# sephiroce/srf

Hardware: AMD Instinct MI355X
Metric: acoustic frames/sec through SRF (123-d fbank, 3-iter DR) at 1/2/4/8 MI355X (higher is better)
Workload: dtype fp32; 1 GPU; wsj_c4: SRF L=6 PH=CH=16 DIM=32 LPAD=RPAD=2 DR iter=3, train step (fwd+bwd+allreduce+Adam); utterances_per_gpu=28, frames_per_utterance=800, global_batch=28, parallelism=dp1, launch=hipgraph (fwd+CTC+bwd)

## Files before the change

### include/srf.h

```cpp
#ifndef SRF_H_
#define SRF_H_
#include <stddef.h>

#ifdef __cplusplus
extern "C" {
#endif

int srf_version(void);
const char* srf_last_error(void);

int srf_route_dr_auto_chunks(int B, int T, int N, int din, int lpad, int rpad, int J, int dout);
int srf_route_dr_split_table(int B, int T, int N, int din, int lpad, int rpad, int J, int dout, int n_chunks,
                             int* info, int* table, int capacity);
int srf_route_dr_set_bal_placement(int on);
int srf_route_dr_split_placement(int B, int T, int N, int din, int lpad, int rpad, int J, int dout, int n_chunks,
                                 int* block_to_wg, int capacity);
size_t srf_route_dr_saved_floats(int B, int T, int J, int dout, int iters);
size_t srf_route_dr_fwd_workspace(int B, int T, int N, int din, int lpad, int rpad, int J, int dout, int iters,
                                  int n_chunks);
size_t srf_route_dr_bwd_workspace(int B, int T, int N, int din, int lpad, int rpad, int J, int dout, int iters,
                                  int n_chunks);
int srf_route_dr_fwd(const float* emb, const float* W, const float* bias, int B, int T, int N, int din, int lpad,
                     int rpad, int J, int dout, int iters, int mask_first, int n_chunks, float* v_out,
                     float* saved, void* workspace, size_t workspace_bytes, void* stream);
size_t srf_route_dr_coupling_floats(int B, int T, int N, int din, int lpad, int rpad, int J, int dout, int iters);
#define SRF_DR_LAYOUT_N 17
int srf_route_dr_operand_layout(int B, int T, int N, int din, int lpad, int rpad, int J, int dout, int iters,
                                long long* out);
int srf_route_dr_fwd_ex(const float* emb, const float* W, const float* bias, int B, int T, int N, int din, int lpad,
                        int rpad, int J, int dout, int iters, int mask_first, int n_chunks, float* v_out,
                        float* saved, float* couplings, void* workspace, size_t workspace_bytes, void* stream);
int srf_route_dr_bwd_ex(const float* emb, const float* W, const float* bias, int B, int T, int N, int din, int lpad,
                        int rpad, int J, int dout, int iters, int mask_first, int n_chunks, const float* saved,
                        const float* couplings, const float* g_v, float* g_emb, float* g_W, float* g_bias,
                        void* workspace, size_t workspace_bytes, void* stream);
int srf_route_dr_bwd_weights_ex(const float* emb, int B, int T, int N, int din, int lpad, int rpad, int J, int dout,
                                int iters, int mask_first, int n_chunks, const float* saved, const float* couplings,
                                float* g_W, float* g_bias, void* workspace, size_t workspace_bytes, void* stream);
int srf_route_dr_bwd_data_ex(const float* emb, const float* W, const float* bias, int B, int T, int N, int din,
                             int lpad, int rpad, int J, int dout, int iters, int mask_first, int n_chunks,
                             const float* saved, const float* couplings, const float* g_v, float* g_emb,
                             void* workspace, size_t workspace_bytes, void* stream);
int srf_set_seed_source(const void* step_counter);
int srf_set_fault_flag(void* flag);
int srf_route_dr_bwd(const float* emb, const float* W, const float* bias, int B, int T, int N, int din, int lpad,
                     int rpad, int J, int dout, int iters, int mask_first, int n_chunks, const float* saved,
                     const float* g_v, float* g_emb, float* g_W, float* g_bias, void* workspace,
                     size_t workspace_bytes, void* stream);
int srf_route_dr_bwd_data(const float* emb, const float* W, const float* bias, int B, int T, int N, int din,
                          int lpad, int rpad, int J, int dout, int iters, int mask_first, int n_chunks,
                          const float* saved, const float* g_v, float* g_emb, void* workspace,
                          size_t workspace_bytes, void* stream);
int srf_route_dr_bwd_weights(const float* emb, int B, int T, int N, int din, int lpad, int rpad, int J, int dout,
                             int iters, int mask_first, int n_chunks, float* g_W, float* g_bias, void* workspace,
                             size_t workspace_bytes, void* stream);

size_t srf_route_sdr_saved_floats(int B, int T, int J, int dout);
size_t srf_route_sdr_fwd_workspace(int B, int T, int N, int din, int lpad, int rpad, int J, int dout);
size_t srf_route_sdr_bwd_workspace(int B, int T, int N, int din, int lpad, int rpad, int J, int dout, int iters);
int srf_route_sdr_fwd(const float* emb, const float* W, const float* bias, int B, int T, int N, int din, int lpad,
                      int rpad, int J, int dout, int iters, int mask_first, float* v_out, float* saved,
                      void* workspace, size_t workspace_bytes, void* stream);
int srf_route_sdr_bwd(const float* emb, const float* W, const float* bias, int B, int T, int N, int din, int lpad,
                      int rpad, int J, int dout, int iters, int mask_first, const float* saved, const float* g_v,
                      float* g_emb, float* g_W, float* g_bias, void* workspace, size_t workspace_bytes,
                      void* stream);

#define SRF_SDR_MAX_ITEMS 8
typedef struct {
// ... 251 lines not shown
```

### srf_amd/_lib.py

```python
import ctypes
import os

_HERE = os.path.dirname(os.path.abspath(__file__))
LIB_PATH = os.environ.get('SRF_LIB_PATH') or os.path.join(_HERE, 'libsrf.so')

_c_int, _c_size, _vp = ctypes.c_int, ctypes.c_size_t, ctypes.c_void_p

SDR_MAX_ITEMS = 8


class SdrRange(ctypes.Structure):
    _fields_ = [('t0', _c_int), ('t1', _c_int), ('emb', _vp), ('W', _vp), ('bias', _vp), ('WT', _vp),
                ('u', _vp), ('v0', _c_int), ('vn', _c_int), ('v', _vp), ('couplings', _vp),
                ('workspace', _vp), ('workspace_bytes', _c_size), ('g_v', _vp), ('carry', _vp),
                ('gu', _vp), ('g0', _c_int), ('gn', _c_int), ('g_emb', _vp), ('g_W', _vp), ('g_bias', _vp),
                ('accumulate', _c_int), ('u_bf16', _c_int), ('group', _c_int), ('gu_factored', _c_int)]


_ranges = ctypes.POINTER(SdrRange)

CAPSNORM_MAX_ITEMS = 8


class CapsnormRange(ctypes.Structure):
    _fields_ = [('t0', _c_int), ('t1', _c_int), ('layer', _c_int), ('x', _vp), ('gamma', _vp), ('beta', _vp),
                ('y', _vp), ('stat', _vp), ('g_y', _vp), ('g_x', _vp), ('gpart', _vp)]


_cn_ranges = ctypes.POINTER(CapsnormRange)

STREAM_ADVANCE_MAX = 32


class StreamBuf(ctypes.Structure):
    _fields_ = [('ptr', _vp), ('row_bytes', _c_size), ('rows_per_stream', _c_int), ('shift', _c_int),
                ('keep', _c_int)]

_SIGNATURES = {
    'srf_version': (_c_int, []),
    'srf_last_error': (ctypes.c_char_p, []),
    'srf_set_seed_source': (_c_int, [_vp]),
    'srf_set_fault_flag': (_c_int, [_vp]),
    'srf_route_dr_auto_chunks': (_c_int, [_c_int] * 8),
    'srf_route_dr_split_table': (_c_int, [_c_int] * 9 + [_vp, _vp, _c_int]),
    'srf_route_dr_set_bal_placement': (_c_int, [_c_int]),
    'srf_route_dr_split_placement': (_c_int, [_c_int] * 9 + [_vp, _c_int]),
    'srf_route_dr_saved_floats': (_c_size, [_c_int] * 5),
    'srf_route_dr_fwd_workspace': (_c_size, [_c_int] * 10),
    'srf_route_dr_bwd_workspace': (_c_size, [_c_int] * 10),
    'srf_route_dr_fwd': (_c_int, [_vp, _vp, _vp] + [_c_int] * 11 + [_vp, _vp, _vp, _c_size, _vp]),
    'srf_route_dr_bwd': (_c_int, [_vp, _vp, _vp] + [_c_int] * 11 + [_vp, _vp, _vp, _vp, _vp, _vp, _c_size, _vp]),
    'srf_route_dr_bwd_data': (_c_int, [_vp, _vp, _vp] + [_c_int] * 11 + [_vp, _vp, _vp, _vp, _c_size, _vp]),
    'srf_route_dr_bwd_weights': (_c_int, [_vp] + [_c_int] * 11 + [_vp, _vp, _vp, _c_size, _vp]),
    'srf_route_dr_coupling_floats': (_c_size, [_c_int] * 9),
    'srf_route_dr_operand_layout': (_c_int, [_c_int] * 9 + [_vp]),
    'srf_route_dr_fwd_ex': (_c_int, [_vp, _vp, _vp] + [_c_int] * 11 + [_vp, _vp, _vp, _vp, _c_size, _vp]),
    'srf_route_dr_bwd_ex': (_c_int, [_vp, _vp, _vp] + [_c_int] * 11 + [_vp] * 7 + [_c_size, _vp]),
    'srf_route_dr_bwd_data_ex': (_c_int, [_vp, _vp, _vp] + [_c_int] * 11 + [_vp] * 5 + [_c_size, _vp]),
    'srf_route_dr_bwd_weights_ex': (_c_int, [_vp] + [_c_int] * 11 + [_vp] * 5 + [_c_size, _vp]),
    'srf_route_sdr_saved_floats': (_c_size, [_c_int] * 4),
    'srf_route_sdr_fwd_workspace': (_c_size, [_c_int] * 8),
    'srf_route_sdr_bwd_workspace': (_c_size, [_c_int] * 9),
    'srf_route_sdr_fwd': (_c_int, [_vp, _vp, _vp] + [_c_int] * 10 + [_vp, _vp, _vp, _c_size, _vp]),
    'srf_route_sdr_bwd': (_c_int, [_vp, _vp, _vp] + [_c_int] * 10 + [_vp, _vp, _vp, _vp, _vp, _vp, _c_size, _vp]),
    'srf_route_sdr_pose': (_c_int, [_vp, _vp, _vp] + [_c_int] * 10 + [_vp, _c_int, _c_int, _vp]),
    'srf_route_sdr_pose_fp8': (_c_int, [_vp, _vp, _vp] + [_c_int] * 10 + [_vp, _c_int, _c_int, _vp]),
    'srf_route_sdr_recur_workspace': (_c_size, [_c_int] * 5),
    'srf_route_sdr_recur_zero_range': (_c_size, [_c_int] * 5 + [ctypes.POINTER(_c_size)]),
    'srf_route_sdr_coupling_floats': (_c_size, [_c_int] * 4),
    'srf_route_sdr_couplings_required': (_c_int, [_c_int] * 4),
    'srf_route_sdr_fact_floats': (_c_size, [_c_int] * 4),
    'srf_route_sdr_recur_fwd': (_c_int, [_vp] + [_c_int] * 11 + [_vp, _vp, _vp, _c_size, _vp]),
    'srf_route_sdr_recur_bwd': (_c_int, [_vp, _c_int, _c_int, _vp, _vp, _vp] + [_c_int] * 9
                                + [_vp, _vp, _c_int, _c_int, _vp, _c_size, _vp]),
    'srf_route_sdr_transpose_w': (_c_int, [_vp] + [_c_int] * 4 + [_vp, _vp]),
    'srf_route_sdr_gx': (_c_int, [_vp, _c_int, _c_int, _vp] + [_c_int] * 10 + [_vp, _vp]),
    'srf_route_sdr_gw': (_c_int, [_vp, _c_int, _c_int, _vp] + [_c_int] * 11 + [_vp, _vp, _vp]),
    'srf_route_sdr_pose_n': (_c_int, [_ranges] + [_c_int] * 10 + [_vp]),
    'srf_route_sdr_recur_fwd_n': (_c_int, [_ranges] + [_c_int] * 8 + [_vp]),
    'srf_route_sdr_recur_bwd_n': (_c_int, [_ranges] + [_c_int] * 8 + [_vp]),
    'srf_route_sdr_gx_n': (_c_int, [_ranges] + [_c_int] * 9 + [_vp]),
    'srf_route_sdr_gw_n': (_c_int, [_ranges] + [_c_int] * 9 + [_vp]),
    'srf_route_sdr_gx_gw_n': (_c_int, [_ranges] + [_c_int] * 9 + [_vp]),
    'srf_route_sdr_gx_gw_fact_n': (_c_int, [_ranges] + [_c_int] * 10 + [_vp]),
    'srf_cnnfe_out_dims': (_c_int, [_c_int, _c_int, ctypes.POINTER(_c_int), ctypes.POINTER(_c_int)]),
    'srf_cnnfe_saved_bytes': (_c_size, [_c_int] * 4),
    'srf_cnnfe_fwd_workspace': (_c_size, [_c_int] * 4),
    'srf_cnnfe_bwd_workspace': (_c_size, [_c_int] * 4),
    'srf_cnnfe_fwd': (_c_int, [_vp, _vp] + [_c_int] * 4 + [_vp] * 16 + [_c_int, ctypes.c_float, ctypes.c_ulonglong,
                                                                       _vp, _vp, _c_size, _vp, _c_size, _vp]),
    'srf_cnnfe_bwd': (_c_int, [_vp, _vp] + [_c_int] * 4 + [_vp] * 4 + [ctypes.c_float, ctypes.c_ulonglong]
                      + [_vp] * 15 + [_c_size, _vp]),
    'srf_cnnfe_bwd_parts': (_c_int, [_c_int, _vp, _vp] + [_c_int] * 4 + [_vp] * 4 + [ctypes.c_float, ctypes.c_ulonglong]
                            + [_vp] * 15 + [_c_size, _vp]),
    'srf_primary_caps_saved_bytes': (_c_size, [_c_int] * 4),
    'srf_primary_caps_bwd_workspace': (_c_size, [_c_int] * 5),
    'srf_primary_caps_fwd': (_c_int, [_vp, _vp] + [_c_int] * 5 + [_vp] * 8 + [_c_int, ctypes.c_float, ctypes.c_float,
                                                                           ctypes.c_ulonglong, _vp, _vp, _c_size, _vp]),
    'srf_primary_caps_bwd': (_c_int, [_vp, _vp] + [_c_int] * 5 + [_vp] * 5 + [_c_int, ctypes.c_float, ctypes.c_float,
# ... 112 lines not shown
```

### srf_amd/csrc/route_dr.hip

```cpp
#include <algorithm>
#include <cmath>
#include <type_traits>

#include "srf_common.h"
#include "route_fwd32.h"
#include "../../include/srf.h"
#include "../../include/srf_prof.h"

namespace {

constexpr float kSquashEps = 1e-7f;

thread_local hipEvent_t* t_ev_start = nullptr;
thread_local hipEvent_t* t_ev_stop = nullptr;
thread_local int t_ev_n = 0;
constexpr int MODE_FWD = 0;
constexpr int MODE_BWD = 1;

using srf::DrGeom;

template <int KS>
__device__ __forceinline__ void load_vec(const float* __restrict__ p, float (&v)[KS]) {
  if constexpr (KS % 4 == 0) {
#pragma unroll
// ... 2350 lines not shown
  const bool bal = p.bal_G > 0;
  const int n_wg = bal ? p.bal_G : p.n_ftiles * p.n_chunks;
  info[0] = bal ? 1 : 0;
  info[1] = n_wg;
  info[2] = p.n_ftiles * in_n;
  info[3] = p.n_slots;
  info[4] = p.plan_arg;
  int n = 0;
  auto emit = [&](int w, int ft, int i0, int i1, int slot) {
    if (n < capacity) {
      int* row = table + (size_t)n * 5;
      row[0] = w, row[1] = ft, row[2] = i0, row[3] = i1, row[4] = slot;
    }
    ++n;
  };
  for (int w = 0; w < n_wg; ++w) {
    if (!bal) {
      const int ft = w / p.n_chunks, slot = w - ft * p.n_chunks;
      const int i0 = slot * p.chunk_len;
      emit(w, ft, std::min(i0, in_n), std::min(in_n, i0 + p.chunk_len), slot);
      continue;
    }
    int u = srf::bal_first(w, p.bal_U, p.bal_G);
    const int u1 = srf::bal_first(w + 1, p.bal_U, p.bal_G);
    while (u < u1) {
      const int ft = u / in_n, i0 = u - ft * in_n, i1 = std::min(in_n, i0 + (u1 - u));
      emit(w, ft, i0, i1, w - srf::bal_owner(ft * in_n, p.bal_U, p.bal_G));
      u += i1 - i0;
    }
  }
  return n;
}

int srf_route_dr_set_bal_placement(int on) {
  srf::fwd32_set_bal_placement(on != 0);
  return SRF_OK;
}

int srf_route_dr_split_placement(int B, int T, int N, int din, int lpad, int rpad, int J, int dout, int n_chunks,
                                 int* block_to_wg, int capacity) {
  const bool shape_ok = B > 0 && T > 0 && N > 0 && lpad >= 0 && rpad >= 0;
  const DrPlan plan = shape_ok ? query(B, T, N, din, lpad, rpad, J, dout, 1, n_chunks) : DrPlan{};
  SRF_REQUIRE(shape_ok && plan.fwd32, "split_placement: not a 32x32-pass shape");
  SRF_REQUIRE(n_chunks == 0 || plan_arg_ok(plan, n_chunks), "split_placement: bad plan argument %d", n_chunks);
  SRF_REQUIRE(capacity >= 0 && (block_to_wg != nullptr || capacity == 0), "split_placement: null argument");
  const srf::Fwd32Plan& p = plan.p32;
  if (p.bal_G <= 0) return 0;
  int d, inv;
  srf::bal_place_params(p.bal_G, p.n_ftiles, srf::fwd32_bal_placement(), &d, &inv);
  for (int b = 0; b < p.bal_G && b < capacity; ++b) block_to_wg[b] = srf::bal_place(b, p.bal_G, d, inv);
  return p.bal_G;
}

size_t srf_route_dr_saved_floats(int B, int T, int J, int dout, int iters) {
  return (size_t)2 * iters * B * T * J * dout;
}

size_t srf_route_dr_fwd_workspace(int B, int T, int N, int din, int lpad, int rpad, int J, int dout, int iters,
                                  int n_chunks) {
  (void)iters;
  return query(B, T, N, din, lpad, rpad, J, dout, 1, n_chunks).fwd_bytes;
}

size_t srf_route_dr_bwd_workspace(int B, int T, int N, int din, int lpad, int rpad, int J, int dout, int iters,
                                  int n_chunks) {
  return query(B, T, N, din, lpad, rpad, J, dout, iters, n_chunks).ws.bytes;
}

size_t srf_route_dr_coupling_floats(int B, int T, int N, int din, int lpad, int rpad, int J, int dout, int iters) {
  const DrPlan p = query(B, T, N, din, lpad, rpad, J, dout, iters, 0);
  return p.can_store ? p.cpl.total : 0;
}

int srf_route_dr_operand_layout(int B, int T, int N, int din, int lpad, int rpad, int J, int dout, int iters,
                                long long* out) {
  SRF_REQUIRE(out != nullptr, "operand_layout: null argument");
  DrPlan p;
  const DrGeom g{B, T, N, din, lpad, rpad, J, dout, iters, 0};
  if (const int rc = check_geom(g)) return rc;
  resolve(p, g, 0, true);
  if (!p.couplings) {
    srf::set_error("operand_layout: no coupling storage for this shape");
    return SRF_EUNSUPPORTED;
  }
  const srf::Fwd32Shape& s = p.p32;
  const size_t in_n = g.in_n(), Fp = padded_frames(g);
  const size_t pl = p.cpl.planes;
  const size_t v[SRF_DR_LAYOUT_N] = {pl,
                                     2 * in_n * s.JDp * g.din * 2,
                                     pl + s.ws_w / 4,
                                     in_n * s.JDp * 8,
                                     pl + (s.ws_w + s.ws_b) / 4,
                                     2 * s.xplane * 2,
                                     pl + (s.ws_w + s.ws_b + s.ws_x) / 4,
                                     3 * sizeof(float),
                                     p.cpl.WT,
                                     in_n * g.din * ((size_t)g.NT() * 16) * 4,
                                     p.cpl.xT,
                                     in_n * g.din * Fp * 4,
                                     (size_t)s.JDp,
                                     s.xplane,
                                     Fp,
                                     p.gx == GxPass::kStored16 ? 1u : 0u,
                                     p.gw == GwPass::kGw16s ? 1u : 0u};
  for (int k = 0; k < SRF_DR_LAYOUT_N; ++k) out[k] = (long long)v[k];
  return SRF_OK;
// ... 78 lines not shown
```

### srf_amd/csrc/route_fwd32.h

```cpp
#pragma once
#include <hip/hip_runtime.h>
#include <cstddef>
#include <cstdint>

namespace srf {

struct DrGeom {
  int B, T, N, din, lpad, rpad, J, dout, iters, mask_first;
  int F() const { return B * T; }
  int in_n() const { return N * (lpad + rpad + 1); }
  int JD() const { return J * dout; }
  int NT() const { return (J * dout + 15) / 16; }
};

constexpr int kFwd32TW = 4;
__host__ __device__ inline int fwd32_frame_stride(int F) { return (F + 31) / 32 * 32; }

__host__ __device__ inline int bal_first(int w, int U, int G) {
  return (int)((uint32_t)w * (uint32_t)U / (uint32_t)G);
}
__host__ __device__ inline int bal_owner(int u, int U, int G) {
  return (int)((((uint32_t)u + 1u) * (uint32_t)G - 1u) / (uint32_t)U);
}
__host__ __device__ inline int bal_tile_slots(int ft, int in_n, int U, int G) {
// ... 3 lines not shown
  if (d == 0) return b;
  const uint32_t x = (uint32_t)b & 7u, k = (uint32_t)b >> 3, q = (uint32_t)G >> 3, rem = (uint32_t)G & 7u;
  const uint32_t r = x * q + (x < rem ? x : rem) + k;
  const uint32_t Gp = (uint32_t)G / (uint32_t)d;
  return (int)((r / (uint32_t)d) * (uint32_t)inv % Gp + (r % (uint32_t)d) * Gp);
}
inline void bal_place_params(int G, int n_ft, bool on, int* d, int* inv) {
  *d = 0, *inv = 0;
  if (!on || G <= 8 || n_ft <= 0) return;
  int a = n_ft, b = G;
  while (b) { const int t = a % b; a = b, b = t; }
  const int Gp = G / a, m = (n_ft / a) % Gp;
  int v = 0;
  for (int c = 0; c < Gp; ++c)
    if ((long long)c * m % Gp == 1 % Gp) { v = c; break; }
  *d = a, *inv = v;
}
void fwd32_set_bal_placement(bool on);
bool fwd32_bal_placement();

constexpr int kBalFlag = 1 << 20;

struct Fwd32Shape {
  int NW;
  int TW;
  int JDp;
  int xpad;
  int n_ftiles;
  size_t xplane;
  size_t ws_w, ws_b, ws_x, ws_h;
};
struct Fwd32Split {
  int n_chunks, chunk_len;
  int bal_G, bal_U;
  int n_slots;
  int plan_arg;
  size_t ws_bsum, ws_slab;
};
struct Fwd32Plan : Fwd32Shape, Fwd32Split {};

bool fwd32_supported(int din, int dout, int J);
Fwd32Plan fwd32_plan(const DrGeom& g, int n_chunks = 0);
size_t fwd32_planes_bytes(const Fwd32Shape& p);
size_t fwd32_scratch_bytes(const Fwd32Split& p);
size_t fwd32_workspace(const Fwd32Plan& p);
size_t fwd32_lds(const Fwd32Shape& p);
float* fwd32_slab(const Fwd32Split& p, void* scratch);
const float* fwd32_hdr(const Fwd32Shape& p, const void* planes);
int fwd32_prepare(const Fwd32Plan& p, const DrGeom& g, const float* emb, const float* W, const float* bias,
                  void* planes, void* scratch, float* WT, float* xT, hipStream_t st, bool wt16 = false,
                  bool xt16 = false);
int fwd32_pass(const Fwd32Plan& p, const DrGeom& g, bool first, const void* planes, void* scratch, const float* vc,
               float* cst, hipStream_t st);
bool fwd32_first_full_supported(const Fwd32Shape& p, const DrGeom& g);
int fwd32_first_full(const Fwd32Plan& p, const DrGeom& g, const void* planes, void* scratch, float* s_out,
                     float* vc_out, float* v_out, hipStream_t st);
struct Fwd32Cpl {
  size_t c, lz, planes, WT, xT, total;
};
Fwd32Cpl fwd32_cpl_layout(const Fwd32Shape& p, const DrGeom& g);
int bwd32_pass(const Fwd32Plan& p, const DrGeom& g, const void* planes, void* scratch, const float* cst,
               const float* gs, float* glst, hipStream_t st);

}
```

### srf_amd/csrc/route_fwd32.hip

```cpp
#include <cmath>
#include <cstdint>
#include <cstdlib>
#include <algorithm>
#include <type_traits>

#include "srf_common.h"
#include "route_fwd32.h"


#ifndef SRF_DR_IL
#define SRF_DR_IL 1
#endif

#ifndef SRF_DR_BAL_AUTO
#define SRF_DR_BAL_AUTO 1
#endif

#ifndef SRF_PREP32_ONEPASS
#define SRF_PREP32_ONEPASS 1
#endif

#ifndef SRF_DR_BAL_XCD
#define SRF_DR_BAL_XCD 1
#endif
// ... 865 lines not shown
#pragma unroll
  for (int t = 0; t < kFTW; ++t)
#pragma unroll
    for (int b = 0; b < kFFB; ++b) acc[t][b] = f16v{};
  auto fetch = [&](int i, FirstFrags<DIN>& fr) {
#pragma unroll
    for (int b = 0; b < kFFB; ++b)
      fetch_x<DIN>(rs, x_voff<DIN>(i, A.N, A.lpad, A.T, A.F, f[b], ftt[b], fv[b], h, A.zero_off), h, A.xplane_b,
                   A.zero_off, fr.b[b]);
#pragma unroll
    for (int t = 0; t < kFTW; ++t) fetch_w<DIN>(rs, wvo + t * TSTEP, h, A.wplane_b, (uint32_t)i * capb, fr.a[t]);
  };
  auto mfmas = [&](const FirstFrags<DIN>& fr) {
#pragma unroll
    for (int t = 0; t < kFTW; ++t)
#pragma unroll
      for (int b = 0; b < kFFB; ++b) acc[t][b] = pose_chain<DIN>(fr.a[t], fr.b[b], acc[t][b]);
  };
  if (i0 < i1) {
    FirstFrags<DIN> f0, f1;
    fetch(i0, f0);
    int i = i0;
    for (; i + 1 < i1; i += 2) {
      fetch(i + 1, f1);
      mfmas(f0);
      if (i + 2 < i1) fetch(i + 2, f0);
      mfmas(f1);
    }
    if (i < i1) mfmas(f0);
  }
  const int Jeff = A.J - (A.mask_first ? 1 : 0);
  const float inv = A.hdr[0];
#pragma unroll
  for (int t = 0; t < kFTW; ++t)
#pragma unroll
    for (int q = 0; q < 4; ++q) {
      const int row = (tbase + t) * 32 + 8 * q + 4 * h;
      const int j = row / DOUT;
      const float c0 = (j < A.J && !(A.mask_first && j == 0)) ? 1.f / (float)Jeff : 0.f;
      if (row < JD) {
        const f4 bsv = *reinterpret_cast<const f4*>(A.bsum + (size_t)chunk * JD + row);
#pragma unroll
        for (int b = 0; b < kFFB; ++b) {
          if (!fv[b]) continue;
          f4 v = {acc[t][b][4 * q], acc[t][b][4 * q + 1], acc[t][b][4 * q + 2], acc[t][b][4 * q + 3]};
          *reinterpret_cast<f4*>(A.slab + ((size_t)chunk * A.F + f[b]) * JD + row) = (v * inv + bsv) * c0;
        }
      }
    }
}

constexpr int kFfBM = 128;
constexpr int kFfA = 2 * kFfBM * 64;
template <int BN>
constexpr int ff_stage() { return kFfA + 2 * BN * 64; }


__device__ __forceinline__ uint32_t ff_slot(int r, int c) { return (uint32_t)(4 * r + (c ^ ((r >> 2) & 3))); }

__device__ __forceinline__ void glds16(const void* src, char* lds_dst) {
  __builtin_amdgcn_global_load_lds((const __attribute__((address_space(1))) void*)src,
                                   (__attribute__((address_space(3))) void*)lds_dst, 16, 0, 0);
}

__device__ __forceinline__ void x_dma(const char* xs, uint32_t xplane_b, uint32_t xvo, int wv, char* dst) {
  const int q = __builtin_amdgcn_readfirstlane(wv) & 3;
  const char* base = xs + (q & 1) * xplane_b + (q >> 1) * 32;
  const uint32_t m0 = __builtin_amdgcn_readfirstlane((uint32_t)reinterpret_cast<uintptr_t>(dst + q * kXlPiece));
  asm volatile("s_mov_b32 m0, %0\n\ts_nop 0\n\tglobal_load_lds_dwordx4 %1, %2" ::"s"(m0), "v"(xvo), "s"(base)
               : "memory", "m0");
}
__device__ __forceinline__ int lane_asm() {
  int lid;
  asm volatile("v_mbcnt_lo_u32_b32 %0, -1, 0\n\tv_mbcnt_hi_u32_b32 %0, -1, %0" : "=v"(lid));
  return lid;
}
template <int K = 0>
__device__ __forceinline__ void xl_wait() {
  asm volatile("s_waitcnt vmcnt(%0)" ::"n"(K) : "memory");
}
__device__ __forceinline__ void xl_wait_all() {
  __builtin_amdgcn_s_waitcnt(0x0F70);
}

template <int BN, int CPS = 1>
__global__ __launch_bounds__(64 * 2 * (BN / 32)) void route_fwd32_first_full_kernel(
    Args32 A, float* __restrict__ s_out, float* __restrict__ vc_out, float* __restrict__ v_out) {
  constexpr int NWF = BN / 32, NWV = 2 * NWF;
  constexpr int NPA = kFfA / 1024, NPB = 2 * BN * 64 / 1024, NP = NPA + NPB;
  constexpr int NPW = (NP + NWV - 1) / NWV;
  constexpr int BPP = BN / 16;
  constexpr int kCap = ff_stage<BN>();
  constexpr int kStage = CPS * kCap;
  extern __shared__ __attribute__((aligned(16))) char smem[];
  const int tid = threadIdx.x, lane = tid & 63, wv = tid >> 6;
  const int r32 = lane & 31, h = lane >> 5;
  const int n_rt = A.JDp / kFfBM;
  int blk = blockIdx.x;
  {
    const int nb = gridDim.x, q = nb >> 3, rem = nb & 7, x = blk & 7, idx = blk >> 3;
    blk = (x < rem ? x * (q + 1) : rem * (q + 1) + (x - rem) * q) + idx;
  }
  const int rt = blk % n_rt, ft = blk / n_rt;
  const int row0 = rt * kFfBM, f0 = ft * BN;
  const int wr = wv / NWF, wc = wv - wr * NWF;
  const char* Wb = static_cast<const char*>(A.Ws);
  const char* Xb = static_cast<const char*>(A.xs);
  const size_t capb = (size_t)A.JDp * 64;
  uint32_t src_o[NPW];
  const char* src_b[NPW];
  bool is_b[NPW], live[NPW];
  int bf_[NPW], btt[NPW];
  bool bok[NPW];
#pragma unroll
  for (int k = 0; k < NPW; ++k) {
    const int q = wv + k * NWV;
    live[k] = q < NP;
    is_b[k] = q >= NPA;
    if (!is_b[k]) {
      const int slot = (q & 7) * 64 + lane, r = slot >> 2, c = (slot & 3) ^ ((r >> 2) & 3);
      src_b[k] = Wb + (size_t)(q >> 3) * A.wplane_b;
      src_o[k] = (uint32_t)((row0 + r) * 64 + c * 16);
      bf_[k] = 0, btt[k] = 0, bok[k] = false;
    } else {
      const int qb = q - NPA;
      const int slot = (qb % BPP) * 64 + lane, r = slot >> 2, c = (slot & 3) ^ ((r >> 2) & 3);
      src_b[k] = Xb + (size_t)(qb / BPP) * A.xplane_b;
      src_o[k] = (uint32_t)(c * 16);
      bf_[k] = f0 + r;
      bok[k] = bf_[k] < A.F;
      const int fc = min(bf_[k], A.F - 1);
      btt[k] = fc - (fc / A.T) * A.T;
    }
  }
  auto stage = [&](int i0, int buf) {
#pragma unroll
    for (int c = 0; c < CPS; ++c) {
      const int i = min(i0 + c, A.in_n - 1);
      char* dst = smem + buf * kStage + c * kCap;
#pragma unroll
      for (int k = 0; k < NPW; ++k) {
        if (!live[k]) continue;
        const int q = wv + k * NWV;
        if (!is_b[k])
          glds16(src_b[k] + (size_t)i * capb + src_o[k], dst + q * 1024);
        else
          glds16(src_b[k] +
                     x_voff<32>(i, A.N, A.lpad, A.T, A.F, bf_[k], btt[k], bok[k] && i0 + c < A.in_n, 0,
                                A.zero_off) +
                     src_o[k],
                 dst + q * 1024);
      }
    }
  };
  auto afrag = [&](const char* base, int t, int plane, int sstep) -> h8 {
    const int r = wr * 64 + t * 32 + r32;
    return *reinterpret_cast<const h8*>(base + plane * (kFfBM * 64) + ff_slot(r, 2 * sstep + h) * 16);
  };
  auto bfrag = [&](const char* base, int plane, int sstep) -> h8 {
    const int r = wc * 32 + r32;
    return *reinterpret_cast<const h8*>(base + kFfA + plane * (BN * 64) + ff_slot(r, 2 * sstep + h) * 16);
  };
  f16v acc[2] = {f16v{}, f16v{}};
  const int n_in = A.in_n;
  stage(0, 0);
  for (int i = 0, buf = 0; i < n_in; i += CPS, buf ^= 1) {
    asm volatile("s_waitcnt vmcnt(0)" ::: "memory");
    __syncthreads();
    if (i + CPS < n_in) stage(i + CPS, buf ^ 1);
    auto frags = [&](const char* base, h8 (&b)[4], h8 (&a)[2][4]) {
#pragma unroll
      for (int s = 0; s < 4; ++s) b[s] = bfrag(base, s & 1, s >> 1);
#pragma unroll
      for (int t = 0; t < 2; ++t)
#pragma unroll
        for (int s = 0; s < 4; ++s) a[t][s] = afrag(base, t, s & 1, s >> 1);
    };
    auto pose2 = [&](const h8 (&a)[2][4], const h8 (&b)[4]) {
      constexpr int ka[6] = {1, 3, 0, 2, 0, 2}, kb[6] = {0, 2, 1, 3, 0, 2};
#pragma unroll
      for (int k = 0; k < 6; ++k)
#pragma unroll
        for (int t = 0; t < 2; ++t) acc[t] = mfma32h(a[t][ka[k]], b[kb[k]], acc[t]);
    };
    const char* base0 = smem + buf * kStage;
    h8 b0[4], a0[2][4];
    frags(base0, b0, a0);
    if constexpr (CPS == 2) {
      h8 b1[4], a1[2][4];
      __builtin_amdgcn_sched_barrier(0);
      frags(base0 + kCap, b1, a1);
      pose2(a0, b0);
#pragma unroll
      for (int k = 0; k < 12; ++k) {
        __builtin_amdgcn_sched_group_barrier(0x008, 1, 0);
        __builtin_amdgcn_sched_group_barrier(0x100, 1, 0);
      }
      __builtin_amdgcn_sched_barrier(0);
      pose2(a1, b1);
    } else {
      pose2(a0, b0);
    }
  }
  const int f = f0 + wc * 32 + r32;
  const bool fv = f < A.F;
  const int JD = A.J * 32;
  const int Jeff = A.J - (A.mask_first ? 1 : 0);
  const float inv = A.hdr[0];
#pragma unroll
  for (int t = 0; t < 2; ++t) {
    const int rbase = row0 + wr * 64 + t * 32;
    const int j = rbase / 32;
    const float c0 = (j < A.J && !(A.mask_first && j == 0)) ? 1.f / (float)Jeff : 0.f;
    f4 sv[4];
    float n2 = 0.f;
#pragma unroll
    for (int q = 0; q < 4; ++q) {
      const int row = rbase + 8 * q + 4 * h;
      f4 bs = {0.f, 0.f, 0.f, 0.f};
      if (row < JD)
        for (int ch = 0; ch < A.n_chunks; ++ch) bs += *reinterpret_cast<const f4*>(A.bsum + (size_t)ch * JD + row);
      const f4 u = {acc[t][4 * q], acc[t][4 * q + 1], acc[t][4 * q + 2], acc[t][4 * q + 3]};
      sv[q] = (u * inv + bs) * c0;
      n2 += (sv[q].x * sv[q].x + sv[q].y * sv[q].y) + (sv[q].z * sv[q].z + sv[q].w * sv[q].w);
    }
    n2 = xor32_sum(n2);
    const float fac = n2 / (1.f + n2) / sqrtf(n2 + 1e-7f);
    if (fv && rbase < JD) {
#pragma unroll
      for (int q = 0; q < 4; ++q) {
        const size_t o = (size_t)f * JD + rbase + 8 * q + 4 * h;
        *reinterpret_cast<f4*>(s_out + o) = sv[q];
        const f4 v = sv[q] * fac;
        *reinterpret_cast<f4*>(vc_out + o) = v;
        if (v_out) *reinterpret_cast<f4*>(v_out + o) = v;
      }
    }
  }
}

template <int DIN, int DOUT, int NW, int TW>
__global__ __launch_bounds__(64 * NW) __attribute__((amdgpu_waves_per_eu(kWavesPerEU))) void route_fwd32_kernel(Args32 A) {
  constexpr int CP = TW * 32 / DOUT;
  constexpr int OWN = CP / 2;
  extern __shared__ __attribute__((aligned(16))) float lds[];
  const int wv = threadIdx.x >> 6;
  const int wvu = __builtin_amdgcn_readfirstlane(wv);
  const int tbase = __builtin_amdgcn_readfirstlane(wv * TW);
  const int j0 = tbase * 32 / DOUT;
  const Rsrc3 rs{make_rsrc(A.Ws, A.ws_bytes), make_rsrc(A.bs, A.bs_bytes), make_rsrc(A.xs, A.xs_bytes)};
  if (DIN <= 16 && NW > 1 && wv >= NW / 2) __builtin_amdgcn_s_setprio(1);
// ... 1155 lines not shown
  Args32 a{};
  a.Ws = base;
  a.bs = base + p.ws_w;
  a.xs = base + p.ws_w + p.ws_b;
  a.hdr = reinterpret_cast<const float*>(base + p.ws_w + p.ws_b + p.ws_x);
  a.ws_bytes = p.ws_w;
  a.bs_bytes = (size_t)in_n * p.JDp * 8;
  a.xs_bytes = 2 * p.xplane * 2;
  a.wplane_b = (uint32_t)((size_t)in_n * p.JDp * g.din * 2);
  a.xplane_b = (uint32_t)(p.xplane * 2);
  a.zero_off = (uint32_t)((p.xplane - p.xpad) * 2);
  a.F = g.F();
  a.T = g.T;
  a.N = g.N;
  a.lpad = g.lpad;
  a.in_n = in_n;
  a.J = g.J;
  a.JDp = p.JDp;
  a.n_chunks = p.n_chunks;
  a.chunk_len = p.chunk_len;
  a.mask_first = g.mask_first;
  a.n_tgroups = p.NW;
  a.vc = nullptr;
  a.bsum = reinterpret_cast<const float*>(scratch);
  a.slab = fwd32_slab(p, scratch);
  a.cst = nullptr;
  a.JP = p.JDp / g.dout;
  a.Fs = fwd32_frame_stride(g.F());
  a.bal_G = p.bal_G;
  a.bal_U = p.bal_U;
  if (p.bal_G > 0) srf::bal_place_params(p.bal_G, p.n_ftiles, fwd32_bal_placement(), &a.bal_d, &a.bal_inv);
  return a;
}

Fwd32Cpl fwd32_cpl_layout(const Fwd32Shape& p, const DrGeom& g) {
  Fwd32Cpl c{};
  const size_t in_n = g.in_n();
  const size_t blk = (size_t)fwd32_frame_stride(g.F()) * in_n;
  const int R1 = std::max(g.iters - 1, 0);
  c.c = 0;
  c.lz = (size_t)R1 * blk * (p.JDp / g.dout);
  size_t off = c.lz + (size_t)R1 * blk;
  off = (off + 63) / 64 * 64;
  c.planes = off;
  off += (fwd32_planes_bytes(p) + 255) / 256 * 64;
  c.WT = off;
  off += (in_n * g.din * ((g.JD() + 15) / 16 * 16) + 63) / 64 * 64;
  c.xT = off;
  off += (in_n * g.din * ((g.F() + 15) / 16 * 16) + 63) / 64 * 64;
  c.total = off;
  return c;
}

bool fwd32_first_full_supported(const Fwd32Shape& p, const DrGeom& g) {
  return g.din == 32 && g.dout == 32 && p.JDp % kFfBM == 0;
}

#ifndef SRF_FF_BN
#define SRF_FF_BN 0
#endif
static int ff_frames(int n_rt, int F) {
  if (SRF_FF_BN) return SRF_FF_BN;
  int dev = 0, cus = 256;
  if (hipGetDevice(&dev) != hipSuccess || hipDeviceGetAttribute(&cus, hipDeviceAttributeMultiprocessorCount, dev) != hipSuccess)
    cus = 256;
  for (int bn : {192, 128, 96})
    if ((long)n_rt * ((F + bn - 1) / bn) >= cus * 9 / 10) return bn;
  return 64;
}

int fwd32_first_full(const Fwd32Plan& p, const DrGeom& g, const void* planes, void* scratch, float* s_out,
                     float* vc_out, float* v_out, hipStream_t st) {
  SRF_REQUIRE(fwd32_first_full_supported(p, g), "fwd32_first_full: din %d dout %d JDp %d", g.din, g.dout, p.JDp);
  SRF_REQUIRE(2 * p.xplane * 2 < (1ull << 31) && p.ws_w < (1ull << 31), "fwd32: operand planes exceed 2 GiB");
  const Args32 a = make_args32(p, g, planes, scratch);
  const int bn = ff_frames(p.JDp / kFfBM, g.F());
  const int nb = (p.JDp / kFfBM) * ((g.F() + bn - 1) / bn);
#define SRF_FF_LAUNCH(BN)                                                                                          \
  if (bn == BN) {                                                                                                 \
    constexpr int CPS_ = BN >= 96 ? 2 : 1;                                                                        \
    const size_t lds = 2 * CPS_ * (size_t)ff_stage<BN>();                                                        \
    if (lds > 64 * 1024)                                                                                          \
      SRF_HIP_TRY(hipFuncSetAttribute((const void*)route_fwd32_first_full_kernel<BN, CPS_>,                       \
                                      hipFuncAttributeMaxDynamicSharedMemorySize, (int)lds));                      \
    hipLaunchKernelGGL((route_fwd32_first_full_kernel<BN, CPS_>), dim3(nb), dim3(64 * 2 * (BN / 32)), lds, st, a, \
                       s_out, vc_out, v_out);                                                                     \
  }
  SRF_FF_LAUNCH(64)
  SRF_FF_LAUNCH(96)
  SRF_FF_LAUNCH(128)
  SRF_FF_LAUNCH(192)
#undef SRF_FF_LAUNCH
  SRF_LAUNCH_CHECK("route_fwd32_first_full");
  return SRF_OK;
}

int fwd32_pass(const Fwd32Plan& p, const DrGeom& g, bool first, const void* planes, void* scratch, const float* vc,
               float* cst, hipStream_t st) {
  Args32 a = make_args32(p, g, planes, scratch);
  a.vc = vc;
  a.cst = first ? nullptr : cst;
  SRF_REQUIRE(2 * p.xplane * 2 < (1ull << 31) && p.ws_w < (1ull << 31), "fwd32: operand planes exceed 2 GiB");
  return dispatch_row(g, "fwd32", [&](auto di, auto dout) {
    if (first) {
      Args32 b = a;
      b.n_tgroups = p.JDp / (32 * kFTW);
      const int tasks = (p.n_ftiles + kFFB - 1) / kFFB * b.n_tgroups * p.n_chunks;
      hipLaunchKernelGGL((route_fwd32_first_kernel<di, dout>), dim3((tasks + 3) / 4), dim3(256), 0, st, b);
      SRF_LAUNCH_CHECK("route_fwd32_first");
      return SRF_OK;
    }
    return dispatch_tiles<di>(p, [&](auto nw, auto tw) {
      return launch_rpass<nw, tw>(p, "route_fwd32", route_fwd32p_kernel<di, dout, (nw > 1 ? nw : 2), (tw <= 2 ? tw : 2)>,
                                  route_fwd32_kernel<di, dout, nw, tw>, st, a);
    });
  });
}

int bwd32_pass(const Fwd32Plan& p, const DrGeom& g, const void* planes, void* scratch, const float* cst,
               const float* gs, float* glst, hipStream_t st) {
  Args32 a = make_args32(p, g, planes, scratch);
  a.mask_first = 0;
  const Bwd32Args b{cst, gs, glst};
  return dispatch_row(g, "bwd32", [&](auto di, auto dout) {
    return dispatch_tiles<di>(p, [&](auto nw, auto tw) {
      return launch_rpass<nw, tw>(p, "route_bwd32", route_bwd32p_kernel<di, dout, (nw > 1 ? nw : 2), (tw <= 2 ? tw : 2)>,
                                  route_bwd32_kernel<di, dout, nw, tw>, st, a, b);
    });
  });
}

}
```

Measured before the change: 3.298 million frames/s.

## Stage each frame window's input image once in LDS and reuse it across taps

The first-full forward pass kernel used to gather one unfolded X tile per input position (window tap). It now loads one padded image of BN+window-1 frames per node into a small ring of LDS images and reads the B fragments for every tap as row-shifted views of it, masking rows that fall outside the utterance. This cuts redundant global-to-LDS traffic for the input operand by roughly the window size, at the cost of extra masking logic and a different LDS footprint. The frames-per-block choice now also checks LDS capacity and can be overridden at runtime through a new API, replacing the compile-time SRF_FF_BN macro.

After: 3.304 million frames/s (median of 6 runs). About the same (+0.2%).

```diff
diff --git a/include/srf.h b/include/srf.h
--- a/include/srf.h
+++ b/include/srf.h
@@ -15,6 +15,8 @@
 int srf_route_dr_set_bal_placement(int on);
 int srf_route_dr_split_placement(int B, int T, int N, int din, int lpad, int rpad, int J, int dout, int n_chunks,
                                  int* block_to_wg, int capacity);
+int srf_route_dr_set_first_full_frames(int bn);
+int srf_route_dr_first_full_frames(int B, int T, int N, int din, int lpad, int rpad, int J, int dout);
 size_t srf_route_dr_saved_floats(int B, int T, int J, int dout, int iters);
 size_t srf_route_dr_fwd_workspace(int B, int T, int N, int din, int lpad, int rpad, int J, int dout, int iters,
                                   int n_chunks);
diff --git a/srf_amd/_lib.py b/srf_amd/_lib.py
--- a/srf_amd/_lib.py
+++ b/srf_amd/_lib.py
@@ -45,6 +45,8 @@
     'srf_route_dr_split_table': (_c_int, [_c_int] * 9 + [_vp, _vp, _c_int]),
     'srf_route_dr_set_bal_placement': (_c_int, [_c_int]),
     'srf_route_dr_split_placement': (_c_int, [_c_int] * 9 + [_vp, _c_int]),
+    'srf_route_dr_set_first_full_frames': (_c_int, [_c_int]),
+    'srf_route_dr_first_full_frames': (_c_int, [_c_int] * 8),
     'srf_route_dr_saved_floats': (_c_size, [_c_int] * 5),
     'srf_route_dr_fwd_workspace': (_c_size, [_c_int] * 10),
     'srf_route_dr_bwd_workspace': (_c_size, [_c_int] * 10),
diff --git a/srf_amd/csrc/route_dr.hip b/srf_amd/csrc/route_dr.hip
--- a/srf_amd/csrc/route_dr.hip
+++ b/srf_amd/csrc/route_dr.hip
@@ -2426,6 +2426,17 @@
   return p.bal_G;
 }
 
+int srf_route_dr_set_first_full_frames(int bn) {
+  SRF_REQUIRE(srf::fwd32_set_first_full_frames(bn), "set_first_full_frames: %d is not 0, 64, 96, 128 or 192", bn);
+  return SRF_OK;
+}
+
+int srf_route_dr_first_full_frames(int B, int T, int N, int din, int lpad, int rpad, int J, int dout) {
+  if (!(B > 0 && T > 0 && N > 0 && lpad >= 0 && rpad >= 0)) return 0;
+  const DrPlan plan = query(B, T, N, din, lpad, rpad, J, dout, 1, 0);
+  return plan.fwd32 ? srf::fwd32_first_full_frames(plan.p32, plan.g) : 0;
+}
+
 size_t srf_route_dr_saved_floats(int B, int T, int J, int dout, int iters) {
   return (size_t)2 * iters * B * T * J * dout;
 }
diff --git a/srf_amd/csrc/route_fwd32.h b/srf_amd/csrc/route_fwd32.h
--- a/srf_amd/csrc/route_fwd32.h
+++ b/srf_amd/csrc/route_fwd32.h
@@ -79,6 +79,8 @@
                   bool xt16 = false);
 int fwd32_pass(const Fwd32Plan& p, const DrGeom& g, bool first, const void* planes, void* scratch, const float* vc,
                float* cst, hipStream_t st);
+bool fwd32_set_first_full_frames(int bn);
+int fwd32_first_full_frames(const Fwd32Shape& p, const DrGeom& g);
 bool fwd32_first_full_supported(const Fwd32Shape& p, const DrGeom& g);
 int fwd32_first_full(const Fwd32Plan& p, const DrGeom& g, const void* planes, void* scratch, float* s_out,
                      float* vc_out, float* v_out, hipStream_t st);
diff --git a/srf_amd/csrc/route_fwd32.hip b/srf_amd/csrc/route_fwd32.hip
--- a/srf_amd/csrc/route_fwd32.hip
+++ b/srf_amd/csrc/route_fwd32.hip
@@ -941,9 +941,23 @@
 
 constexpr int kFfBM = 128;
 constexpr int kFfA = 2 * kFfBM * 64;
-template <int BN>
-constexpr int ff_stage() { return kFfA + 2 * BN * 64; }
-
+constexpr int kFfLdsMax = 160 * 1024;
+constexpr int ff_cps(int bn) { return bn >= 96 ? 2 : 1; }
+__host__ __device__ constexpr int ff_img_rows(int bn, int wn) { return (bn + wn - 1 + 15) / 16 * 16; }
+__host__ __device__ constexpr int ff_n_img(int cps, int wn) { return (2 * cps - 2) / wn + 2; }
+__host__ __device__ constexpr size_t ff_lds(int bn, int wn) {
+  return (size_t)2 * ff_cps(bn) * kFfA + (size_t)ff_n_img(ff_cps(bn), wn) * ff_img_rows(bn, wn) * 128;
+}
+
+struct FfPos {
+  int n, w, ib;
+  __device__ __forceinline__ void next(int Wn, int n_img) {
+    if (++w == Wn) {
+      w = 0, ++n;
+      if (++ib == n_img) ib = 0;
+    }
+  }
+};
 
 __device__ __forceinline__ uint32_t ff_slot(int r, int c) { return (uint32_t)(4 * r + (c ^ ((r >> 2) & 3))); }
 
@@ -976,13 +990,12 @@
 __global__ __launch_bounds__(64 * 2 * (BN / 32)) void route_fwd32_first_full_kernel(
     Args32 A, float* __restrict__ s_out, float* __restrict__ vc_out, float* __restrict__ v_out) {
   constexpr int NWF = BN / 32, NWV = 2 * NWF;
-  constexpr int NPA = kFfA / 1024, NPB = 2 * BN * 64 / 1024, NP = NPA + NPB;
-  constexpr int NPW = (NP + NWV - 1) / NWV;
-  constexpr int BPP = BN / 16;
-  constexpr int kCap = ff_stage<BN>();
-  constexpr int kStage = CPS * kCap;
+  constexpr int NPA = CPS * (kFfA / 1024);
+  constexpr int NKA = (NPA + NWV - 1) / NWV;
+  constexpr int ROT = NWV - NPA % NWV;
+  constexpr int kStage = CPS * kFfA;
   extern __shared__ __attribute__((aligned(16))) char smem[];
-  const int tid = threadIdx.x, lane = tid & 63, wv = tid >> 6;
+  const int tid = threadIdx.x, lane = tid & 63, wv = __builtin_amdgcn_readfirstlane(tid >> 6);
   const int r32 = lane & 31, h = lane >> 5;
   const int n_rt = A.JDp / kFfBM;
   int blk = blockIdx.x;
@@ -996,75 +1009,89 @@
   const char* Wb = static_cast<const char*>(A.Ws);
   const char* Xb = static_cast<const char*>(A.xs);
   const size_t capb = (size_t)A.JDp * 64;
-  uint32_t src_o[NPW];
-  const char* src_b[NPW];
-  bool is_b[NPW], live[NPW];
-  int bf_[NPW], btt[NPW];
-  bool bok[NPW];
-#pragma unroll
-  for (int k = 0; k < NPW; ++k) {
-    const int q = wv + k * NWV;
-    live[k] = q < NP;
-    is_b[k] = q >= NPA;
-    if (!is_b[k]) {
-      const int slot = (q & 7) * 64 + lane, r = slot >> 2, c = (slot & 3) ^ ((r >> 2) & 3);
-      src_b[k] = Wb + (size_t)(q >> 3) * A.wplane_b;
-      src_o[k] = (uint32_t)((row0 + r) * 64 + c * 16);
-      bf_[k] = 0, btt[k] = 0, bok[k] = false;
-    } else {
-      const int qb = q - NPA;
-      const int slot = (qb % BPP) * 64 + lane, r = slot >> 2, c = (slot & 3) ^ ((r >> 2) & 3);
-      src_b[k] = Xb + (size_t)(qb / BPP) * A.xplane_b;
-      src_o[k] = (uint32_t)(c * 16);
-      bf_[k] = f0 + r;
-      bok[k] = bf_[k] < A.F;
-      const int fc = min(bf_[k], A.F - 1);
-      btt[k] = fc - (fc / A.T) * A.T;
-    }
-  }
-  auto stage = [&](int i0, int buf) {
+  const int Wn = A.in_n / A.N;
+  const int IPP = ff_img_rows(BN, Wn) / 16;
+  const int kImgP = IPP * 1024, kImg = 2 * kImgP;
+  const int n_img = ff_n_img(CPS, Wn);
+  char* const imgs = smem + 2 * kStage;
+  const int lr = lane >> 2, lc = (lane & 3) ^ ((lane >> 4) & 3);
+  const uint32_t lo = (uint32_t)(lr * 64 + lc * 16);
+  auto stage = [&](FfPos& d, int buf) {
+    int ic[CPS];
 #pragma unroll
     for (int c = 0; c < CPS; ++c) {
-      const int i = min(i0 + c, A.in_n - 1);
-      char* dst = smem + buf * kStage + c * kCap;
-#pragma unroll
-      for (int k = 0; k < NPW; ++k) {
-        if (!live[k]) continue;
-        const int q = wv + k * NWV;
-        if (!is_b[k])
-          glds16(src_b[k] + (size_t)i * capb + src_o[k], dst + q * 1024);
-        else
-          glds16(src_b[k] +
-                     x_voff<32>(i, A.N, A.lpad, A.T, A.F, bf_[k], btt[k], bok[k] && i0 + c < A.in_n, 0,
-                                A.zero_off) +
-                     src_o[k],
-                 dst + q * 1024);
-      }
+      ic[c] = min(d.w * A.N + d.n, A.in_n - 1);
+      if (d.w == 0 && d.n < A.N) {
+        char* dst = imgs + d.ib * kImg;
+        const int rbase = f0 - A.lpad;
+        for (int q = (wv + ROT) % NWV; q < 2 * IPP; q += NWV) {
+          const int pl = q >= IPP ? 1 : 0, pr = (q - pl * IPP) * 16;
+          const int fs = rbase + pr + lr;
+          const uint32_t vo = (fs >= 0 && fs < A.F) ? (uint32_t)((d.n * A.F + rbase + pr) * 64) + lo
+                                                    : A.zero_off + (uint32_t)(lc * 16);
+          glds16(Xb + (size_t)pl * A.xplane_b + vo, dst + q * 1024);
+        }
+      }
+      d.next(Wn, n_img);
+    }
+    char* dst = smem + buf * kStage;
+#pragma unroll
+    for (int k = 0; k < NKA; ++k) {
+      const int q = wv + k * NWV;
+      if (q >= NPA) continue;
+      const int i = CPS == 2 && (q >> 4) ? ic[CPS - 1] : ic[0];
+      glds16(Wb + (size_t)((q >> 3) & 1) * A.wplane_b + (size_t)i * capb + (uint32_t)(row0 * 64 + (q & 7) * 1024) + lo,
+             dst + q * 1024);
     }
   };
+  const int rb = wc * 32 + r32;
+  int wlo, awlo, awhi;
+  {
+    const int f = f0 + rb;
+    const int fc = min(f, A.F - 1);
+    wlo = f < A.F ? A.lpad - (fc - (fc / A.T) * A.T) : (1 << 30);
+    int hi = wlo, lw = wlo;
+#pragma unroll
+    for (int m = 32; m; m >>= 1) {
+      hi = max(hi, __shfl_xor(hi, m));
+      lw = min(lw, __shfl_xor(lw, m));
+    }
+    awlo = __builtin_amdgcn_readfirstlane(hi);
+    awhi = __builtin_amdgcn_readfirstlane(lw) + A.T;
+  }
   auto afrag = [&](const char* base, int t, int plane, int sstep) -> h8 {
     const int r = wr * 64 + t * 32 + r32;
     return *reinterpret_cast<const h8*>(base + plane * (kFfBM * 64) + ff_slot(r, 2 * sstep + h) * 16);
   };
-  auto bfrag = [&](const char* base, int plane, int sstep) -> h8 {
-    const int r = wc * 32 + r32;
-    return *reinterpret_cast<const h8*>(base + kFfA + plane * (BN * 64) + ff_slot(r, 2 * sstep + h) * 16);
+  auto bfrags = [&](const FfPos& c, h8 (&b)[4]) {
+    const char* img = imgs + c.ib * kImg;
+    const int r = rb + c.w;
+    const uint32_t o0 = (uint32_t)(r << 6) | (uint32_t)((((r >> 2) & 3) ^ h) << 4), o1 = o0 ^ 32u;
+    b[0] = *reinterpret_cast<const h8*>(img + o0);
+    b[1] = *reinterpret_cast<const h8*>(img + kImgP + o0);
+    b[2] = *reinterpret_cast<const h8*>(img + o1);
+    b[3] = *reinterpret_cast<const h8*>(img + kImgP + o1);
+  };
+  auto afrags = [&](const char* base, h8 (&a)[2][4]) {
+#pragma unroll
+    for (int t = 0; t < 2; ++t)
+#pragma unroll
+      for (int s = 0; s < 4; ++s) a[t][s] = afrag(base, t, s & 1, s >> 1);
+  };
+  auto mask = [&](const FfPos& c, h8 (&b)[4]) {
+    if (c.n < A.N && c.w >= awlo && c.w < awhi) return;
+    const bool ok = c.n < A.N && (uint32_t)(c.w - wlo) < (uint32_t)A.T;
+#pragma unroll
+    for (int s = 0; s < 4; ++s) b[s] = ok ? b[s] : h8{};
   };
   f16v acc[2] = {f16v{}, f16v{}};
   const int n_in = A.in_n;
-  stage(0, 0);
+  FfPos pd{0, 0, 0}, pc{0, 0, 0};
+  stage(pd, 0);
   for (int i = 0, buf = 0; i < n_in; i += CPS, buf ^= 1) {
     asm volatile("s_waitcnt vmcnt(0)" ::: "memory");
     __syncthreads();
-    if (i + CPS < n_in) stage(i + CPS, buf ^ 1);
-    auto frags = [&](const char* base, h8 (&b)[4], h8 (&a)[2][4]) {
-#pragma unroll
-      for (int s = 0; s < 4; ++s) b[s] = bfrag(base, s & 1, s >> 1);
-#pragma unroll
-      for (int t = 0; t < 2; ++t)
-#pragma unroll
-        for (int s = 0; s < 4; ++s) a[t][s] = afrag(base, t, s & 1, s >> 1);
-    };
+    if (i + CPS < n_in) stage(pd, buf ^ 1);
     auto pose2 = [&](const h8 (&a)[2][4], const h8 (&b)[4]) {
       constexpr int ka[6] = {1, 3, 0, 2, 0, 2}, kb[6] = {0, 2, 1, 3, 0, 2};
 #pragma unroll
@@ -1074,11 +1101,15 @@
     };
     const char* base0 = smem + buf * kStage;
     h8 b0[4], a0[2][4];
-    frags(base0, b0, a0);
+    bfrags(pc, b0);
+    afrags(base0, a0);
+    mask(pc, b0);
+    pc.next(Wn, n_img);
     if constexpr (CPS == 2) {
       h8 b1[4], a1[2][4];
       __builtin_amdgcn_sched_barrier(0);
-      frags(base0 + kCap, b1, a1);
+      bfrags(pc, b1);
+      afrags(base0 + kFfA, a1);
       pose2(a0, b0);
 #pragma unroll
       for (int k = 0; k < 12; ++k) {
@@ -1086,6 +1117,8 @@
         __builtin_amdgcn_sched_group_barrier(0x100, 1, 0);
       }
       __builtin_amdgcn_sched_barrier(0);
+      mask(pc, b1);
+      pc.next(Wn, n_img);
       pose2(a1, b1);
     } else {
       pose2(a0, b0);
@@ -2347,39 +2380,45 @@
   return c;
 }
 
-bool fwd32_first_full_supported(const Fwd32Shape& p, const DrGeom& g) {
-  return g.din == 32 && g.dout == 32 && p.JDp % kFfBM == 0;
-}
-
-#ifndef SRF_FF_BN
-#define SRF_FF_BN 0
-#endif
-static int ff_frames(int n_rt, int F) {
-  if (SRF_FF_BN) return SRF_FF_BN;
+static int g_ff_frames = 0;
+bool fwd32_set_first_full_frames(int bn) {
+  if (bn != 0 && bn != 64 && bn != 96 && bn != 128 && bn != 192) return false;
+  g_ff_frames = bn;
+  return true;
+}
+
+int fwd32_first_full_frames(const Fwd32Shape& p, const DrGeom& g) {
+  if (g.din != 32 || g.dout != 32 || p.JDp % kFfBM != 0) return 0;
+  const int wn = g.lpad + g.rpad + 1;
+  auto fits = [&](int bn) { return ff_lds(bn, wn) <= (size_t)kFfLdsMax; };
+  if (g_ff_frames) return fits(g_ff_frames) ? g_ff_frames : 0;
   int dev = 0, cus = 256;
   if (hipGetDevice(&dev) != hipSuccess || hipDeviceGetAttribute(&cus, hipDeviceAttributeMultiprocessorCount, dev) != hipSuccess)
     cus = 256;
+  const long n_rt = p.JDp / kFfBM;
   for (int bn : {192, 128, 96})
-    if ((long)n_rt * ((F + bn - 1) / bn) >= cus * 9 / 10) return bn;
-  return 64;
-}
+    if (n_rt * ((g.F() + bn - 1) / bn) >= cus * 9 / 10 && fits(bn)) return bn;
+  return fits(64) ? 64 : 0;
+}
+
+bool fwd32_first_full_supported(const Fwd32Shape& p, const DrGeom& g) { return fwd32_first_full_frames(p, g) != 0; }
 
 int fwd32_first_full(const Fwd32Plan& p, const DrGeom& g, const void* planes, void* scratch, float* s_out,
                      float* vc_out, float* v_out, hipStream_t st) {
-  SRF_REQUIRE(fwd32_first_full_supported(p, g), "fwd32_first_full: din %d dout %d JDp %d", g.din, g.dout, p.JDp);
+  const int bn = fwd32_first_full_frames(p, g);
+  SRF_REQUIRE(bn != 0, "fwd32_first_full: din %d dout %d JDp %d window %d", g.din, g.dout, p.JDp, g.lpad + g.rpad + 1);
   SRF_REQUIRE(2 * p.xplane * 2 < (1ull << 31) && p.ws_w < (1ull << 31), "fwd32: operand planes exceed 2 GiB");
   const Args32 a = make_args32(p, g, planes, scratch);
-  const int bn = ff_frames(p.JDp / kFfBM, g.F());
   const int nb = (p.JDp / kFfBM) * ((g.F() + bn - 1) / bn);
-#define SRF_FF_LAUNCH(BN)                                                                                          \
-  if (bn == BN) {                                                                                                 \
-    constexpr int CPS_ = BN >= 96 ? 2 : 1;                                                                        \
-    const size_t lds = 2 * CPS_ * (size_t)ff_stage<BN>();                                                        \
-    if (lds > 64 * 1024)                                                                                          \
-      SRF_HIP_TRY(hipFuncSetAttribute((const void*)route_fwd32_first_full_kernel<BN, CPS_>,                       \
-                                      hipFuncAttributeMaxDynamicSharedMemorySize, (int)lds));                      \
+  const size_t lds = ff_lds(bn, g.lpad + g.rpad + 1);
+#define SRF_FF_LAUNCH(BN)                                                                                        \
+  if (bn == BN) {                                                                                               \
+    constexpr int CPS_ = ff_cps(BN);                                                                            \
+    if (lds > 64 * 1024)                                                                                        \
+      SRF_HIP_TRY(hipFuncSetAttribute((const void*)route_fwd32_first_full_kernel<BN, CPS_>,                     \
+                                      hipFuncAttributeMaxDynamicSharedMemorySize, (int)lds));                    \
     hipLaunchKernelGGL((route_fwd32_first_full_kernel<BN, CPS_>), dim3(nb), dim3(64 * 2 * (BN / 32)), lds, st, a, \
-                       s_out, vc_out, v_out);                                                                     \
+                       s_out, vc_out, v_out);                                                                   \
   }
   SRF_FF_LAUNCH(64)
   SRF_FF_LAUNCH(96)
```
